# spacejam/loghisto

Measured on AMD Instinct MI355X. Metric: float64 samples/sec bucketed (1 GPU) + % HBM roofline; p99 extract latency, higher is better.
Workload: dtype f64; 1 GPU; C2 single-metric float64 stream, one ingest kernel + one percentile scan per step; distribution=lognormal, metrics=1, ranks=1, merge=none, prewarm=25 untimed K1 launches before the W warm-up steps (clock ramp after idle), input_memory=hipMalloc (lh_tool_device_alloc), not torch's caching allocator

## Files before the change

### include/loghisto_gpu_tuning.h

```cpp
#ifndef LOGHISTO_GPU_TUNING_H
#define LOGHISTO_GPU_TUNING_H

#include "loghisto_gpu.h"

#ifdef __cplusplus
extern "C" {
#endif

enum {
    LH_OPT_TWO_LEVEL_ABOVE = 1,
    LH_OPT_HOT_MIN_TILES = 2,
    LH_OPT_HOT_WINDOWS = 3,
    LH_OPT_NAMES_PER_PARTITION = 4,
    LH_OPT_SMALL_PATH = 8,
    LH_OPT_PART_V2 = 9,
    LH_OPT_PART_V2_MIN_PAIRS = 10,
    LH_OPT_PART_V2_SHAPE = 11,
    LH_OPT_PART_V3 = 12,
    LH_OPT_PART_V3_MIN_PAIRS = 13,
    LH_OPT_PART_V3_LOG_W = 14,
    LH_OPT_PART_MIN_PAIRS = 17,
    LH_OPT_FAIL_SCRATCH_ALLOCS = 19,
    LH_OPT_LANE_GEN3 = 20,
    LH_OPT_PART_V3_DIRECT_MAX_PAIRS = 21,
    LH_OPT_WIDEN_AT_SAMPLES = 23
};

typedef struct lh_dispatch_query {
    uint32_t struct_size;
    uint32_t max_metrics;
    uint64_t n;
    uint64_t ids_addr;
    uint64_t vals_addr;
    uint32_t id_width;
    uint32_t host_fed;
    uint32_t num_cus;
    uint32_t lane_blocks;
    uint64_t lane_samples;
    uint32_t small_disabled, regions_disabled, v3_disabled;
    uint32_t call_log_w;
    uint64_t scratch_cap;
    uint64_t sublaunch_pairs;
    uint64_t part_min_pairs, v2_min_pairs, v3_min_pairs;
    uint32_t v2_off, v3_off, hot_off;
    uint32_t v2_shape_set, v2_shape;
    uint32_t fail_allocs;
    uint32_t lane_gen3_off;
} lh_dispatch_query;

typedef struct lh_dispatch_step {
    uint32_t path;
    uint32_t lane_block;
    uint64_t take;
    uint64_t scratch;
    uint32_t fell_back;
    uint32_t peeled;
} lh_dispatch_step;

int lh_dispatch_probe(const lh_dispatch_query *q, lh_dispatch_step *steps, size_t cap, size_t *nsteps);

int lh_tool_device_alloc(size_t bytes, void **d_ptr);
int lh_tool_device_free(void *d_ptr);
int lh_tool_read_ceiling(const void *d_ptr, size_t bytes, int reps, void *stream, float *avg_ms, float *min_ms);
int lh_tool_last_extract_ms(lh_engine *e, float *kernel_ms, float *copy_ms);
int lh_tool_count_le_switch(uint32_t wave_from_rows, uint32_t *previous);

#ifdef __cplusplus
}
#endif
#endif
```

### loghisto_amd/_native.py

```python
from __future__ import annotations

import ctypes as C
import os

_HERE = os.path.dirname(os.path.abspath(__file__))
LIB_PATH = os.path.join(_HERE, "liblhgpu.so")

ABI_VERSION = 7
ALLOW_OLDER_ABI = False
NKEYS = 65536
NTHRESH = 70980
MAX_PERCENTILES = 32
MAX_BOUNDS = 64
LE_PER_METRIC = 1

OK, EINVAL, ENOMEM, EDEVICE, ENODEVICE, EBUSY, ERANGE, ESTATE = range(8)


class LhConfig(C.Structure):
    _fields_ = [("struct_size", C.c_uint32), ("device", C.c_int32), ("max_metrics", C.c_uint32),
                ("num_buffers", C.c_uint32), ("num_lanes", C.c_uint32), ("max_counters", C.c_uint32),
                ("lane_samples", C.c_uint64), ("cell_bits", C.c_uint32), ("reserved0", C.c_uint32)]


class LhCounters(C.Structure):
    _fields_ = [(k, C.c_uint64) for k in ("samples_single", "samples_small", "samples_partitioned", "samples_direct",
                                           "launches", "flips", "flips_busy", "extracts", "backpressure_waits",
                                           "window_misses")] + [("small_path_disabled", C.c_uint32),
                                                                ("regions_disabled", C.c_uint32),
                                                                ("scratch_bytes", C.c_uint64),
                                                                ("sublaunches", C.c_uint64),
                                                                ("samples_partitioned_v2", C.c_uint64),
                                                                ("counter_events", C.c_uint64),
                                                                ("region_overflows", C.c_uint64),
                                                                ("samples_partitioned_v3", C.c_uint64),
                                                                ("window_log2", C.c_uint64),
                                                                ("records_level1", C.c_uint64),
                                                                ("records_level2", C.c_uint64),
                                                                ("level2_overflows", C.c_uint64),
                                                                ("reduce_window_misses", C.c_uint64),
                                                               ("surveys_reused", C.c_uint64),
                                                               ("scratch_alloc_failures", C.c_uint64),
                                                               ("samples_fallback", C.c_uint64),
                                                               ("survey_stale_pairs", C.c_uint64),
                                                               ("lane_scratch_bytes", C.c_uint64),
                                                               ("widenings", C.c_uint64),
                                                               ("store_bytes", C.c_uint64)]

OPT_TWO_LEVEL_ABOVE, OPT_HOT_MIN_TILES, OPT_HOT_WINDOWS, OPT_NAMES_PER_PARTITION = 1, 2, 3, 4
OPT_EXTRACT_ZERO_COPY, OPT_SCRATCH_CAP_BYTES, OPT_SUBLAUNCH_PAIRS, OPT_SMALL_PATH = 5, 6, 7, 8
OPT_PART_V2, OPT_PART_V2_MIN_PAIRS, OPT_PART_V2_SHAPE = 9, 10, 11
OPT_PART_V3, OPT_PART_V3_MIN_PAIRS, OPT_PART_V3_LOG_W = 12, 13, 14
OPT_LANE_ZERO_COPY = 15
OPT_SURVEY_EVERY = 16
OPT_PART_MIN_PAIRS = 17
OPT_LANE_SCRATCH_BLOCKS = 18
OPT_FAIL_SCRATCH_ALLOCS = 19
OPT_LANE_GEN3 = 20
OPT_PART_V3_DIRECT_MAX_PAIRS = 21
OPT_MERGE_NARROW_CELLS = 22
OPT_WIDEN_AT_SAMPLES = 23


class LhDispatchQuery(C.Structure):
    _fields_ = [("struct_size", C.c_uint32), ("max_metrics", C.c_uint32), ("n", C.c_uint64), ("ids_addr", C.c_uint64),
                ("vals_addr", C.c_uint64), ("id_width", C.c_uint32), ("host_fed", C.c_uint32), ("num_cus", C.c_uint32),
                ("lane_blocks", C.c_uint32), ("lane_samples", C.c_uint64), ("small_disabled", C.c_uint32),
                ("regions_disabled", C.c_uint32), ("v3_disabled", C.c_uint32), ("call_log_w", C.c_uint32),
                ("scratch_cap", C.c_uint64), ("sublaunch_pairs", C.c_uint64), ("part_min_pairs", C.c_uint64),
                ("v2_min_pairs", C.c_uint64), ("v3_min_pairs", C.c_uint64), ("v2_off", C.c_uint32), ("v3_off", C.c_uint32),
                ("hot_off", C.c_uint32), ("v2_shape_set", C.c_uint32), ("v2_shape", C.c_uint32), ("fail_allocs", C.c_uint32),
                ("lane_gen3_off", C.c_uint32)]


class LhDispatchStep(C.Structure):
    _fields_ = [("path", C.c_uint32), ("lane_block", C.c_uint32), ("take", C.c_uint64), ("scratch", C.c_uint64),
                ("fell_back", C.c_uint32), ("peeled", C.c_uint32)]


PATH_DIRECT, PATH_SMALL, PATH_GEN1, PATH_GEN2, PATH_GEN3 = range(5)


class LhExtractView(C.Structure):
    _fields_ = [("stats", C.c_void_p), ("pvals", C.c_void_p), ("pkeys", C.c_void_p), ("pvalid", C.c_void_p),
                ("nmetrics", C.c_size_t), ("np", C.c_size_t)]


class LhExtractCompact(C.Structure):
    _fields_ = [("count", C.c_void_p), ("sum", C.c_void_p), ("nbuckets", C.c_void_p), ("pvalid_bits", C.c_void_p),
                ("pkeys", C.c_void_p), ("nmetrics", C.c_size_t), ("np", C.c_size_t)]


class LhMergeInfo(C.Structure):
    _fields_ = [("packed_cells", C.c_uint64), ("send_bytes", C.c_uint64), ("recv_bytes", C.c_uint64),
                ("widest_row", C.c_uint32), ("occupied_rows", C.c_uint32), ("padded_words", C.c_uint64),
                ("cell_bytes", C.c_uint32), ("rows_8bit", C.c_uint32), ("ranges_ms", C.c_float), ("plan_ms", C.c_float),
                ("pack_ms", C.c_float), ("collective_ms", C.c_float), ("unpack_ms", C.c_float), ("span_ms", C.c_float),
                ("packed_words", C.c_uint64), ("rows_16bit", C.c_uint32), ("reserved", C.c_uint32)]


class LhLineFormat(C.Structure):
    _fields_ = [("prefix", C.c_char_p), ("sep", C.c_char_p), ("suffix", C.c_char_p),
                ("flags", C.c_uint32), ("reserved", C.c_uint32)]


FMT_UNDERSCORE_TO_DOT = 1
SER_AGGREGATES = 1
FMT_SLOT = 336


class LhStats(C.Structure):
    _fields_ = [("count", C.c_uint64), ("sum", C.c_double), ("avg", C.c_double),
                ("agg_sum_add", C.c_uint64), ("nbuckets", C.c_uint32), ("present", C.c_uint32)]


_vp, _sz = C.c_void_p, C.c_size_t
_dp, _u32p, _u64p = C.POINTER(C.c_double), C.POINTER(C.c_uint32), C.POINTER(C.c_uint64)
_i16p, _u8p = C.POINTER(C.c_int16), C.POINTER(C.c_uint8)

TUNING_SIGNATURES = {
    "lh_dispatch_probe": (C.c_int, [C.POINTER(LhDispatchQuery), C.POINTER(LhDispatchStep), _sz, C.POINTER(_sz)]),
    "lh_tool_device_alloc": (C.c_int, [_sz, C.POINTER(_vp)]),
    "lh_tool_device_free": (C.c_int, [_vp]),
    "lh_tool_read_ceiling": (C.c_int, [_vp, _sz, C.c_int, _vp, C.POINTER(C.c_float), C.POINTER(C.c_float)]),
    "lh_tool_last_extract_ms": (C.c_int, [_vp, C.POINTER(C.c_float), C.POINTER(C.c_float)]),
    "lh_tool_count_le_switch": (C.c_int, [C.c_uint32, _u32p]),
}

SIGNATURES = {
    "lh_abi_version": (C.c_int, []),
    "lh_strerror": (C.c_char_p, [C.c_int]),
    "lh_last_error": (C.c_char_p, []),
    "lh_default_config": (C.c_int, [C.POINTER(LhConfig)]),
    "lh_create": (C.c_int, [C.POINTER(LhConfig), C.POINTER(_vp)]),
    "lh_destroy": (C.c_int, [_vp]),
    "lh_intern": (C.c_int, [_vp, C.c_char_p, _sz, _u32p]),
    "lh_lookup": (C.c_int, [_vp, C.c_char_p, _sz, _u32p]),
    "lh_num_metrics": (C.c_int, [_vp, _u32p]),
    "lh_metric_name": (C.c_int, [_vp, C.c_uint32, C.c_char_p, _sz, C.POINTER(_sz)]),
    "lh_submit": (C.c_int, [_vp, C.c_uint32, _vp, _sz]),
    "lh_submit_pairs": (C.c_int, [_vp, _vp, _vp, _sz]),
    "lh_reserve_pairs": (C.c_int, [_vp, _sz, C.POINTER(C.c_void_p), C.POINTER(C.c_void_p), C.POINTER(C.c_size_t),
                                   C.POINTER(C.c_uint32)]),
    "lh_commit_pairs": (C.c_int, [_vp, C.c_uint32, _sz]),
    "lh_submit_pairs16": (C.c_int, [_vp, _vp, _vp, _sz]),
    "lh_reserve_pairs16": (C.c_int, [_vp, _sz, C.POINTER(C.c_void_p), C.POINTER(C.c_void_p), C.POINTER(C.c_size_t),
                                     C.POINTER(C.c_uint32)]),
    "lh_commit_pairs16": (C.c_int, [_vp, C.c_uint32, _sz]),
    "lh_submit_pairs16_device": (C.c_int, [_vp, _vp, _vp, _sz, _vp]),
    "lh_submit_device": (C.c_int, [_vp, C.c_uint32, _vp, _sz, _vp]),
    "lh_submit_pairs_device": (C.c_int, [_vp, _vp, _vp, _sz, _vp]),
    "lh_intern_counter": (C.c_int, [_vp, C.c_char_p, _sz, _u32p]),
    "lh_num_counters": (C.c_int, [_vp, _u32p]),
    "lh_counter_name": (C.c_int, [_vp, C.c_uint32, C.c_char_p, _sz, C.POINTER(_sz)]),
    "lh_submit_counts": (C.c_int, [_vp, _vp, _vp, _sz]),
    "lh_submit_counts_device": (C.c_int, [_vp, _vp, _vp, _sz, _vp]),
    "lh_counters_collect": (C.c_int, [_vp, C.c_uint32, _sz, _u64p, _u8p, _u64p, _u8p]),
    "lh_serialize_counters": (C.c_int, [_vp, C.c_uint32, _sz, C.POINTER(LhLineFormat), _vp, _sz, C.POINTER(_sz)]),
    "lh_flush": (C.c_int, [_vp]),
    "lh_sync": (C.c_int, [_vp]),
    "lh_flip": (C.c_int, [_vp, C.POINTER(_vp)]),
    "lh_extract": (C.c_int, [_vp, _dp, _sz, C.POINTER(LhStats), _dp, _i16p, _u8p, _sz]),
    "lh_extract_rows": (C.c_int, [_vp, C.c_uint32, _sz, _dp, _sz, C.POINTER(LhStats), _dp, _i16p, _u8p]),
    "lh_extract_rows_view": (C.c_int, [_vp, C.c_uint32, _sz, _dp, _sz, C.POINTER(LhExtractView)]),
    "lh_extract_rows_compact": (C.c_int, [_vp, C.c_uint32, _sz, _dp, _sz, C.POINTER(LhExtractCompact)]),
    "lh_expand_compact": (C.c_int, [_vp, C.POINTER(LhExtractCompact), C.POINTER(LhStats), _dp, _i16p, _u8p]),
    "lh_buckets": (C.c_int, [_vp, C.c_uint32, _i16p, _u64p, _sz, C.POINTER(_sz)]),
    "lh_buckets_all": (C.c_int, [_vp, C.c_uint32, _sz, _u64p, _i16p, _u64p, _sz, C.POINTER(_sz)]),
    "lh_snapshot_rows": (C.c_int, [_vp, C.POINTER(_vp), _u32p]),
    "lh_row_stride": (C.c_size_t, []),
    "lh_snapshot_cells": (C.c_int, [_vp, C.POINTER(_vp), _u32p, _u32p]),
    "lh_cell_bytes": (C.c_int, [_vp]),
    "lh_snapshot_ranges": (C.c_int, [_vp, C.POINTER(_vp)]),
    "lh_snapshot_mark_dirty": (C.c_int, [_vp, C.c_uint32, C.c_uint32, C.c_uint32, C.c_uint32]),
    "lh_snapshot_add_buckets": (C.c_int, [_vp, _vp, _vp, _vp, _sz]),
    "lh_snapshot_add_buckets_csr": (C.c_int, [_vp, C.c_uint32, _sz, _vp, _vp, _vp]),
    "lh_snapshot_add_buckets_device": (C.c_int, [_vp, _vp, _vp, _vp, _sz]),
    "lh_snapshot_add_buckets_csr_device": (C.c_int, [_vp, C.c_uint32, _sz, _vp, _vp, _vp]),
    "lh_count_le": (C.c_int, [_vp, C.c_uint32, _sz, _vp, _sz, C.c_uint32, _vp, _vp]),
    "lh_count_le_device": (C.c_int, [_vp, C.c_uint32, _sz, _vp, _sz, C.c_uint32, _vp, _vp]),
    "lh_snapshot_merge": (C.c_int, [_vp, _vp, C.c_int, C.c_int, C.c_int, C.c_uint32, _u32p, _u32p]),
    "lh_snapshot_merge_info": (C.c_int, [_vp, C.POINTER(LhMergeInfo)]),
    "lh_set_rccl_library": (C.c_int, [C.c_char_p]),
    "lh_serialize": (C.c_int, [_vp, C.c_uint32, _sz, _dp, C.POINTER(C.c_char_p), _sz, C.POINTER(LhLineFormat),
                               C.c_uint32, _vp, _sz, C.POINTER(_sz)]),
    "lh_snapshot_accumulate": (C.c_int, [_vp]),
    "lh_lifetime": (C.c_int, [_vp, C.c_uint32, _sz, _u64p, _u64p]),
    "lh_format_f": (C.c_int, [_vp, _dp, _sz, _vp, _sz, _u32p]),
    "lh_snapshot_stream": (C.c_int, [_vp, C.POINTER(_vp)]),
    "lh_release": (C.c_int, [_vp]),
    "lh_get_counters": (C.c_int, [_vp, C.POINTER(LhCounters)]),
    "lh_set_option": (C.c_int, [_vp, C.c_int, C.c_uint64]),
    "lh_compress_device": (C.c_int, [_vp, _vp, _vp, _sz, _vp]),
    "lh_compress_device_golog": (C.c_int, [_vp, _vp, _vp, _sz, _vp]),
    "lh_codec_tables": (C.c_int, [_vp, _dp, _dp]),
    "lh_selftest_vlog": (C.c_int, [_vp, _dp]),
}

_lib = None


class NativeLibraryError(RuntimeError):
    pass


class LhError(RuntimeError):
    def __init__(self, code: int, where: str, detail: str = ""):
        self.code = code
        msg = f"{where}: {lib().lh_strerror(code).decode()} (code {code})"
        if detail:
            msg += f" [{detail}]"
        super().__init__(msg)


def lib():
    global _lib
    if _lib is not None:
        return _lib
    if not os.path.exists(LIB_PATH):
        raise NativeLibraryError(
            f"{LIB_PATH} is missing: build it with `python -m loghisto_amd.build` "
            "(hipcc, gfx950). loghisto_amd has no CPU path.")
    import torch
    try:
        L = C.CDLL(LIB_PATH)
    except OSError as exc:
        raise NativeLibraryError(f"cannot load {LIB_PATH}: {exc}") from exc
    for name, (res, args) in list(SIGNATURES.items()) + list(TUNING_SIGNATURES.items()):
        try:
            fn = getattr(L, name)
        except AttributeError as exc:
            if ALLOW_OLDER_ABI:
                continue
            raise NativeLibraryError(f"{LIB_PATH} does not export {name}") from exc
        fn.restype = res
        fn.argtypes = args
    if L.lh_abi_version() != ABI_VERSION and not (ALLOW_OLDER_ABI and L.lh_abi_version() >= 5):
        raise NativeLibraryError(f"ABI mismatch: library {L.lh_abi_version()}, binding {ABI_VERSION}")
    _lib = L
    return L


def check(code: int, where: str):
    if code != OK:
        detail = lib().lh_last_error().decode() if code in (EDEVICE, ENODEVICE, ENOMEM) else ""
        raise LhError(code, where, detail)
```

### loghisto_amd/build.py

```python
from __future__ import annotations

import os
import shutil
import subprocess
import sys

_HERE = os.path.dirname(os.path.abspath(__file__))
CSRC = os.path.join(_HERE, "csrc")
INCLUDE = os.path.join(os.path.dirname(_HERE), "include")
LIB = os.path.join(_HERE, "liblhgpu.so")

_COMMON = ["-O3", "-std=c++17", "-fPIC", "-ffp-contract=off", "-fno-fast-math", "-Wall", "-Wextra",
           "-Wno-unused-parameter"]
_UNITS = [
    ("lh_kernels.hip", ["--offload-arch=gfx950"]),
    ("lh_kernels_part.hip", ["--offload-arch=gfx950"]),
    ("lh_kernels_small.hip", ["--offload-arch=gfx950"]),
    ("lh_kernels_fmt.hip", ["--offload-arch=gfx950"]),
    ("lh_tools.hip", ["--offload-arch=gfx950"]),
    ("lh_import.hip", ["--offload-arch=gfx950"]),
    ("lh_count.hip", ["--offload-arch=gfx950"]),
    ("lh_engine.cc", []),
    ("lh_dispatch.cc", []),
    ("host/metric_system.cc", []),
]

_PROGRAMS = [
    ("tests/cpp/metrics_test.cc", "metrics_test"),
    ("tools/c5_driver.cc", "c5_driver"),
    ("tools/wire_bench.cc", "wire_bench"),
    ("tools/latency.cc", "latency"),
    ("tools/hostfed_native.cc", "hostfed_native"),
]


_HIP_PROGRAMS = [
    ("tools/read_ceiling.hip", "read_ceiling"),
    ("tools/valu_rates.hip", "valu_rates"),
    ("tools/row_stride.hip", "row_stride"),
]


def _hipcc() -> str:
    for c in (shutil.which("hipcc"), "/opt/rocm/bin/hipcc"):
        if c and os.path.exists(c):
            return c
    raise RuntimeError("hipcc not found; liblhgpu.so cannot be built")


def _stale(target: str, deps) -> bool:
    if not os.path.exists(target):
        return True
    t = os.path.getmtime(target)
    return any(os.path.getmtime(d) > t for d in deps)


def build_native(force: bool = False, verbose: bool = False) -> str:
    hipcc = _hipcc()
    bdir = os.path.join(_HERE, "build")
    os.makedirs(bdir, exist_ok=True)
    headers = [os.path.join(CSRC, f) for f in os.listdir(CSRC) if f.endswith(".h")]
    headers += [os.path.join(INCLUDE, "loghisto_gpu.h"), os.path.join(INCLUDE, "loghisto.hpp")]
    objs = []
    for src, extra in _UNITS:
        s = os.path.join(CSRC, src)
        o = os.path.join(bdir, os.path.splitext(src)[0].replace("/", "_") + ".o")
        if force or _stale(o, [s] + headers):
            cmd = [hipcc] + _COMMON + extra + os.environ.get("LH_EXTRA_CXXFLAGS", "").split() + ["-I", INCLUDE, "-c", s, "-o", o]
            if verbose:
                print(" ".join(cmd), file=sys.stderr)
            subprocess.check_call(cmd)
        objs.append(o)
    if force or _stale(LIB, objs):
        cmd = [hipcc, "-shared", "-fPIC", "-o", LIB] + objs
        if verbose:
            print(" ".join(cmd), file=sys.stderr)
        subprocess.check_call(cmd)
    root = os.path.dirname(_HERE)
    for src, name in _PROGRAMS:
        s = os.path.join(root, src)
        if not os.path.exists(s):
            continue
        out = os.path.join(bdir, name)
        if force or _stale(out, [s, LIB] + headers):
            cmd = ["g++", "-O2", "-std=c++17", "-pthread", "-Wall", "-I", INCLUDE, s, "-o", out,
                   "-L", _HERE, "-llhgpu", "-Wl,-rpath," + _HERE, "-Wl,-rpath,$ORIGIN/.."]
            if verbose:
                print(" ".join(cmd), file=sys.stderr)
            subprocess.check_call(cmd)
    dsrc = os.path.join(root, "tests", "cpp", "dispatch_test.cc")
    if os.path.exists(dsrc):
        out = os.path.join(bdir, "dispatch_test")
        if force or _stale(out, [dsrc, LIB, os.path.join(CSRC, "lh_dispatch.cc")] + headers):
            rocm = os.path.dirname(os.path.dirname(os.path.realpath(hipcc)))
            cmd = ["g++", "-O1", "-std=c++17", "-Wall", "-D__HIP_PLATFORM_AMD__", "-I", os.path.join(rocm, "include"),
                   dsrc, "-o", out, "-L", _HERE, "-llhgpu", "-Wl,-rpath," + _HERE, "-Wl,-rpath,$ORIGIN/..",
                   "-L", os.path.join(rocm, "lib"), "-Wl,-rpath," + os.path.join(rocm, "lib")]
            if verbose:
                print(" ".join(cmd), file=sys.stderr)
            subprocess.check_call(cmd)
    for src, name in _HIP_PROGRAMS:
        s = os.path.join(root, src)
        if not os.path.exists(s):
            continue
        out = os.path.join(bdir, name)
        if force or _stale(out, [s]):
            cmd = [hipcc, "-O3", "-std=c++17", "--offload-arch=gfx950", s, "-o", out]
            if verbose:
                print(" ".join(cmd), file=sys.stderr)
            subprocess.check_call(cmd)
    stub_src = os.path.join(root, "tests", "cpp", "rccl_stub.cc")
    if os.path.exists(stub_src):
        out = os.path.join(bdir, "librccl_stub.so")
        if force or _stale(out, [stub_src]):
            rocm = os.path.dirname(os.path.dirname(os.path.realpath(hipcc)))
            cmd = ["g++", "-O2", "-std=c++17", "-shared", "-fPIC", "-pthread", "-Wall", "-D__HIP_PLATFORM_AMD__",
                   "-I", os.path.join(rocm, "include"), stub_src, "-o", out, "-L", os.path.join(rocm, "lib"),
                   "-lamdhip64"]
            if verbose:
                print(" ".join(cmd), file=sys.stderr)
            subprocess.check_call(cmd)
    return LIB


if __name__ == "__main__":
    print(build_native(force="--force" in sys.argv, verbose=True))
```

Baseline: 789.7 billion samples/s.

## Add windowed LDS histogram ingest kernel with wave aggregation and overflow bins

Replaces the single-metric ingest kernel with a new one. Each workgroup samples its tile to pick a centred LDS bin window, keeps two padded copies of that window to spread atomic contention, and adds two small overflow windows before falling back to global cell adds. Wave-level ballot aggregation merges runs of identical bins into a single atomic, and loads are 16-byte nontemporal. The previous kernel stays reachable through a runtime selector. The window heuristic adds complexity and risks global atomic traffic when a tile's bins spread beyond the windows.

```diff
diff --git a/include/loghisto_gpu_tuning.h b/include/loghisto_gpu_tuning.h
--- a/include/loghisto_gpu_tuning.h
+++ b/include/loghisto_gpu_tuning.h
@@ -64,6 +64,7 @@
 int lh_tool_read_ceiling(const void *d_ptr, size_t bytes, int reps, void *stream, float *avg_ms, float *min_ms);
 int lh_tool_last_extract_ms(lh_engine *e, float *kernel_ms, float *copy_ms);
 int lh_tool_count_le_switch(uint32_t wave_from_rows, uint32_t *previous);
+int lh_tool_k1_select(int which);
 
 #ifdef __cplusplus
 }
diff --git a/loghisto_amd/_native.py b/loghisto_amd/_native.py
--- a/loghisto_amd/_native.py
+++ b/loghisto_amd/_native.py
@@ -125,6 +125,7 @@
     "lh_tool_read_ceiling": (C.c_int, [_vp, _sz, C.c_int, _vp, C.POINTER(C.c_float), C.POINTER(C.c_float)]),
     "lh_tool_last_extract_ms": (C.c_int, [_vp, C.POINTER(C.c_float), C.POINTER(C.c_float)]),
     "lh_tool_count_le_switch": (C.c_int, [C.c_uint32, _u32p]),
+    "lh_tool_k1_select": (C.c_int, [C.c_int]),
 }
 
 SIGNATURES = {
diff --git a/loghisto_amd/build.py b/loghisto_amd/build.py
--- a/loghisto_amd/build.py
+++ b/loghisto_amd/build.py
@@ -13,7 +13,8 @@
 _COMMON = ["-O3", "-std=c++17", "-fPIC", "-ffp-contract=off", "-fno-fast-math", "-Wall", "-Wextra",
            "-Wno-unused-parameter"]
 _UNITS = [
-    ("lh_kernels.hip", ["--offload-arch=gfx950"]),
+    ("lh_kernels.hip", ["--offload-arch=gfx950", "-Dlaunch_ingest_single=launch_ingest_single_r06"]),
+    ("lh_k1.hip", ["--offload-arch=gfx950"]),
     ("lh_kernels_part.hip", ["--offload-arch=gfx950"]),
     ("lh_kernels_small.hip", ["--offload-arch=gfx950"]),
     ("lh_kernels_fmt.hip", ["--offload-arch=gfx950"]),
diff --git a/loghisto_amd/csrc/lh_k1.hip b/loghisto_amd/csrc/lh_k1.hip
--- /dev/null
+++ b/loghisto_amd/csrc/lh_k1.hip
@@ -0,0 +1,218 @@
+#include "lh_kernels.h"
+#include "lh_codec.h"
+#include "../../include/loghisto_gpu_tuning.h"
+
+#include <atomic>
+
+namespace lh {
+
+hipError_t launch_ingest_single_r06(const double *d_v, size_t n, uint64_t *row, uint32_t *range, const double *d_Tx,
+                                    int num_cus, hipStream_t s);
+
+namespace {
+
+typedef double d2_t __attribute__((ext_vector_type(2)));
+
+constexpr int K1_BLOCK = 512;
+constexpr int K1_UNROLL = 8;
+constexpr uint32_t K1_COPIES = 2;
+constexpr uint32_t K1_WIN = 16384 / K1_COPIES;
+constexpr uint32_t K1_PAD = 16;
+constexpr uint32_t K1_STRIDE = K1_WIN + K1_PAD;
+constexpr uint32_t K1_OVF = 1024;
+constexpr uint32_t K1_OVF_NONE = 0xffffffffu;
+constexpr uint32_t K1_MAIN_WORDS = K1_STRIDE * K1_COPIES;
+constexpr uint32_t K1_CTL_WORDS = 8;
+constexpr size_t K1_LDS_BYTES = (size_t)(K1_MAIN_WORDS + 2 * K1_OVF + K1_CTL_WORDS) * sizeof(uint32_t);
+constexpr uint32_t K1_WIDE = K1_WIN * K1_COPIES;
+constexpr uint32_t K1_AGG_MIN = 24;
+static_assert(2 * K1_LDS_BYTES + 2048 <= 160 * 1024, "two workgroups per CU");
+static_assert(K1_OVF >= 64 && K1_OVF <= K1_WIN, "anchor arithmetic");
+static_assert(K1_WIDE <= K1_MAIN_WORDS, "the wide window lies in the copies' words");
+
+__device__ __forceinline__ void global_cell_add(uint64_t *row, uint32_t *s_rng, uint32_t bin, uint32_t c)
+{
+    lh::cell_add_hidden(row, bin, c);
+    if (bin < s_rng[0]) atomicMin(&s_rng[0], bin);
+    if (bin > s_rng[1]) atomicMax(&s_rng[1], bin);
+}
+
+__device__ __forceinline__ uint32_t k1_anchor(uint32_t bin, uint32_t win_lo, uint32_t win_len)
+{
+    const uint32_t centred = bin >= K1_OVF / 2 ? bin - K1_OVF / 2 : 0u, win_hi = win_lo + win_len;
+    if (bin >= win_hi) return min(bin < win_hi + K1_OVF ? win_hi : centred, (uint32_t)LH_NKEYS - K1_OVF);
+    const uint32_t below = win_lo >= K1_OVF ? win_lo - K1_OVF : 0u;
+    return bin >= below ? below : centred;
+}
+
+__device__ __forceinline__ void k1_miss(uint32_t *h0, uint32_t win_lo, uint32_t win_len, uint64_t *row, uint32_t *s_rng,
+                                        uint32_t bin, uint32_t c)
+{
+    const uint32_t side = bin >= win_lo + win_len ? 1u : 0u;
+    uint32_t *anchor = h0 + K1_MAIN_WORDS + 2 * K1_OVF + 2 + side;
+    uint32_t lo = __atomic_load_n(anchor, __ATOMIC_RELAXED);
+    if (lo == K1_OVF_NONE) {
+        const uint32_t want = k1_anchor(bin, win_lo, win_len);
+        const uint32_t seen = atomicCAS(anchor, K1_OVF_NONE, want);
+        lo = seen == K1_OVF_NONE ? want : seen;
+    }
+    const uint32_t rel = bin - lo;
+    if (rel < K1_OVF) atomicAdd(&h0[K1_MAIN_WORDS + side * K1_OVF + rel], c);
+    else global_cell_add(row, s_rng, bin, c);
+}
+
+struct K1Win {
+    uint32_t *h0;
+    uint32_t win_lo, win_len;
+};
+
+__device__ __forceinline__ void k1_add(const K1Win w, uint32_t *hc, uint64_t *row, uint32_t *s_rng, uint32_t bin, uint32_t c = 1u)
+{
+    const uint32_t rel = bin - w.win_lo;
+    if (rel < w.win_len) atomicAdd(&hc[rel], c);
+    else k1_miss(w.h0, w.win_lo, w.win_len, row, s_rng, bin, c);
+}
+
+__device__ __forceinline__ void k1_add_fullwave(const K1Win w, uint32_t *hc, uint64_t *row, uint32_t *s_rng, uint32_t bin)
+{
+    const uint32_t first = __builtin_amdgcn_readfirstlane(bin);
+    const unsigned long long same = __builtin_amdgcn_ballot_w64(bin == first);
+    const uint32_t nsame = (uint32_t)__builtin_popcountll(same);
+    if (nsame >= K1_AGG_MIN) {
+        const bool leader = __lane_id() == 0;
+        if (leader || bin != first) k1_add(w, hc, row, s_rng, bin, leader ? nsame : 1u);
+    } else {
+        k1_add(w, hc, row, s_rng, bin);
+    }
+}
+
+}
+
+__global__ __launch_bounds__(K1_BLOCK) void k_ingest_single2(const double *__restrict__ v, size_t n,
+                                                             uint64_t *__restrict__ row,
+                                                             uint32_t *__restrict__ range,
+                                                             const double *__restrict__ Tx)
+{
+    extern __shared__ __attribute__((aligned(16))) unsigned char smem[];
+    uint32_t *h0 = reinterpret_cast<uint32_t *>(smem);
+    uint32_t *s_ctl = h0 + K1_MAIN_WORDS + 2 * K1_OVF;
+    const uint32_t tid = threadIdx.x;
+
+    const size_t head = (((uintptr_t)v & 8) && n) ? 1 : 0;
+    const d2_t *vp = reinterpret_cast<const d2_t *>(v + head);
+    const size_t npair = (n - head) / 2;
+    const size_t tile = (size_t)K1_BLOCK * K1_UNROLL;
+    const size_t nfull = npair / tile;
+
+    for (uint32_t i = tid; i < K1_MAIN_WORDS + 2 * K1_OVF; i += K1_BLOCK) h0[i] = 0;
+    if (tid < 64) {
+        const size_t i0 = min(head + (size_t)blockIdx.x * tile * 2 + (size_t)tid * (tile * 2 / 64), n - 1);
+        const uint32_t b = lh_bin_of(v[i0], Tx);
+        uint32_t lowest = b, highest = b;
+#pragma unroll
+        for (int d = 32; d >= 1; d >>= 1) {
+            lowest = min(lowest, (uint32_t)__shfl_xor(lowest, d, 64));
+            highest = max(highest, (uint32_t)__shfl_xor(highest, d, 64));
+        }
+        if (tid == 0) {
+            s_ctl[0] = 0xffffffffu;
+            s_ctl[1] = 0;
+            s_ctl[2] = s_ctl[3] = K1_OVF_NONE;
+            const uint32_t len = highest - lowest < K1_WIN - K1_WIN / 8 ? K1_WIN : K1_WIDE;
+            const uint32_t mid = lowest + (highest - lowest) / 2;
+            s_ctl[4] = min(mid >= len / 2 ? mid - len / 2 : 0u, (uint32_t)LH_NKEYS - len);
+            s_ctl[5] = len;
+        }
+    }
+    __syncthreads();
+    const K1Win w = {h0, (uint32_t)__builtin_amdgcn_readfirstlane((int)s_ctl[4]),
+                     (uint32_t)__builtin_amdgcn_readfirstlane((int)s_ctl[5])};
+    uint32_t *h = h0 + (w.win_len == K1_WIN ? (tid % K1_COPIES) * K1_STRIDE : 0u);
+
+    for (size_t t = blockIdx.x; t < nfull; t += gridDim.x) {
+        const d2_t *p = vp + t * tile + tid;
+        d2_t r[K1_UNROLL];
+#pragma unroll
+        for (int u = 0; u < K1_UNROLL; u++) r[u] = __builtin_nontemporal_load(p + u * K1_BLOCK);
+#pragma unroll
+        for (int u = 0; u < K1_UNROLL; u++) {
+            k1_add_fullwave(w, h, row, s_ctl, lh_bin_of(r[u].x, Tx));
+            k1_add_fullwave(w, h, row, s_ctl, lh_bin_of(r[u].y, Tx));
+        }
+    }
+    if (blockIdx.x == nfull % gridDim.x) {
+        for (size_t i = nfull * tile + tid; i < npair; i += K1_BLOCK) {
+            const d2_t x = vp[i];
+            k1_add(w, h, row, s_ctl, lh_bin_of(x.x, Tx));
+            k1_add(w, h, row, s_ctl, lh_bin_of(x.y, Tx));
+        }
+        if (tid == 0 && head) k1_add(w, h, row, s_ctl, lh_bin_of(v[0], Tx));
+        if (tid == 1 && ((n - head) & 1)) k1_add(w, h, row, s_ctl, lh_bin_of(v[n - 1], Tx));
+    }
+    __syncthreads();
+
+    uint32_t lmin = 0xffffffffu, lmax = 0;
+    for (uint32_t i = tid; i < w.win_len; i += K1_BLOCK) {
+        uint32_t c = h0[i];
+        if (w.win_len == K1_WIN) {
+#pragma unroll
+            for (uint32_t k = 1; k < K1_COPIES; k++) c += h0[k * K1_STRIDE + i];
+        }
+        if (c) {
+            lh::cell_add(row, w.win_lo + i, c);
+            lmin = min(lmin, w.win_lo + i);
+            lmax = max(lmax, w.win_lo + i);
+        }
+    }
+    for (uint32_t side = 0; side < 2; side++) {
+        const uint32_t ovf_lo = s_ctl[2 + side];
+        if (ovf_lo == K1_OVF_NONE) continue;
+        for (uint32_t i = tid; i < K1_OVF; i += K1_BLOCK) {
+            const uint32_t c = h0[K1_MAIN_WORDS + side * K1_OVF + i];
+            if (c) {
+                lh::cell_add(row, ovf_lo + i, c);
+                lmin = min(lmin, ovf_lo + i);
+                lmax = max(lmax, ovf_lo + i);
+            }
+        }
+    }
+    if (lmin != 0xffffffffu) { atomicMin(&s_ctl[0], lmin); atomicMax(&s_ctl[1], lmax); }
+    __syncthreads();
+    if (tid == 0 && s_ctl[0] != 0xffffffffu) {
+        atomicMin(&range[0], s_ctl[0]);
+        atomicMax(&range[1], s_ctl[1]);
+    }
+}
+
+namespace {
+std::atomic<int> g_k1_select{0};
+}
+
+hipError_t launch_ingest_single(const double *d_v, size_t n, uint64_t *row, uint32_t *range,
+                                const double *d_Tx, int num_cus, hipStream_t s)
+{
+    if (g_k1_select.load(std::memory_order_relaxed) == 1) return launch_ingest_single_r06(d_v, n, row, range, d_Tx, num_cus, s);
+    if (n == 0) return hipSuccess;
+    static std::atomic<bool> attr_set{false};
+    if (!attr_set) {
+        hipError_t e = hipFuncSetAttribute(reinterpret_cast<const void *>(k_ingest_single2),
+                                           hipFuncAttributeMaxDynamicSharedMemorySize, (int)K1_LDS_BYTES);
+        if (e != hipSuccess) return e;
+        attr_set = true;
+    }
+    const size_t tile_samples = (size_t)K1_BLOCK * K1_UNROLL * 2;
+    size_t want = (n + tile_samples - 1) / tile_samples;
+    size_t cap = (size_t)num_cus * 2;
+    unsigned grid = (unsigned)(want < cap ? want : cap);
+    if (grid == 0) grid = 1;
+    hipLaunchKernelGGL(k_ingest_single2, dim3(grid), dim3(K1_BLOCK), K1_LDS_BYTES, s, d_v, n, row, range, d_Tx);
+    return hipGetLastError();
+}
+
+}
+
+extern "C" int lh_tool_k1_select(int which)
+{
+    if (which != 0 && which != 1) return lh::g_k1_select.load(std::memory_order_relaxed);
+    return lh::g_k1_select.exchange(which, std::memory_order_relaxed);
+}
```

Result: slower. 747.0 billion samples/s (-5.4%).
